# succinctlabs/kzg-rs

Hardware: AMD Instinct MI355X
Metric: blobs/sec verify_blob_kzg_proof_batch (higher is better)
Workload: dtype u32 limbs (255-bit Fr / 381-bit Fp modular integers); 1 GPU; verify_blob_kzg_proof_batch, batches of 1024 synthetic blobs (4096 Fr each), device-resident, known-tau test setup (BASELINE.json configs[1]); one step = one launch group of 256 independent batches = 262144 blobs per GPU; blobs_per_gpu_per_batch=1024, batch=1024, parallelism=shard-by-blob x1, groups_in_flight=4

## Files before the change

### kzg_rs_amd/csrc/capi_verify.hpp

```cpp

static KzgRet launch_evaluate(const KzgSettings* s, const void* d_blobs, const Fr* d_z, Fr* d_y, uint32_t* d_status, size_t T, bool alone = false,
                              bool stamp = false) {
    unsigned long long* const kt = stamp && s->ws.d_ktime ? s->ws.d_ktime + 4 : nullptr;
    if (T > s->eval_scratch_cap) {
        if (s->d_eval_scratch) HIPCHK(hipFree(s->d_eval_scratch));
        s->d_eval_scratch = nullptr;
        s->eval_scratch_cap = 0;
        const size_t cap = T < 1024 ? 1024 : T;
        HIPCHK(hipMalloc(&s->d_eval_scratch, 4 * (size_t)EVAL_SCRATCH_WORDS * cap));
        s->eval_scratch_cap = cap;
    }
    const unsigned per_lane = (unsigned)((T + 63) / 64);
    hipLaunchKernelGGL(k_eval_powers, dim3(per_lane), dim3(64), 0, s->s1, d_z, s->d_eval_scratch, (int)T);
    const unsigned eval_blocks = (unsigned)((T + EVAL_BLOBS_PER_BLOCK - 1) / EVAL_BLOBS_PER_BLOCK);
    static const long pad_opt = ab_int("eval_lds_pad", -1);
    const size_t lds_pad = pad_opt >= 0 ? (size_t)std::min(120L * 1024, pad_opt) : alone ? 0 : 16384;
    size_t spread_lds = eval_blocks <= (unsigned)s->n_cus ? (size_t)EVAL_SPREAD_LDS : lds_pad;
    if (spread_lds && DYN_LDS(k_blob_evaluate_t<true>, spread_lds) != hipSuccess) {
        (void)hipGetLastError();
        spread_lds = 0;
    }
    hipLaunchKernelGGL(k_blob_evaluate_t<true>, dim3(eval_blocks), dim3(64 * EVAL_BLOBS_PER_BLOCK), spread_lds, s->s1,
                       (const uint8_t*)d_blobs, EvalTables{s->d_eval_a, s->d_eval_b, s->d_eval_c}, s->d_eval_scratch, d_status, (int)T, kt);
    hipLaunchKernelGGL(k_eval_finish, dim3(per_lane), dim3(64), 0, s->s1, s->d_eval_scratch, d_y, (int)T);
// ... 127 lines not shown
    MsmDesc d{};
    d.mult = w.d_mult;
    d.pflag = w.d_pflag;
    d.scalars = w.d_scalars;
    d.term_point = w.d_term_point;
    d.term_scalar = w.d_term_scalar;
    d.sorted = w.d_sorted;
    d.window_sums = w.d_window;
    d.nterms[0] = (int)n;
    d.nterms[1] = (int)(2 * n + 1);
    d.max_terms = mt;
    d.stride = 2 * T + 1;
    d.ktime = w.kstamps_valid ? w.d_ktime + 8 : nullptr;
    d.chunks = w.chunks;
    d.chunks_per_block = w.chunks == MSM_CHUNKS ? msm_chunks_per_block(B) : 1;
    static const int msm_flags = ab_flag("msm_xcd", true) ? MSM_FLAG_XCD : 0;
    d.flags = msm_flags;
    const unsigned slots = d.chunks / d.chunks_per_block, W = MSM_WINDOWS / d.chunks;
    unsigned S = 1;
    while (S < MSM_MAX_SLICES && W * slots * 2 * B * S < 768 && n / (2 * S) >= 1024 && 2 * S * B <= 128) S *= 2;
    static const unsigned latency_slices = [] {
        const unsigned v = (unsigned)ab_int("msm_latency_slices", 0);
        return v == 1 || v == 2 || v == 4 || v == 8 ? v : 4u;
    }();
    if (d.chunks != MSM_CHUNKS && S == 1 && n >= 256 && B <= 4) S = latency_slices;
    const size_t lds_cap = msm_lds_sort_capacity<Curve29>();
    auto slice_terms = [&](unsigned S_) { return ((size_t)mt + S_ - 1) / S_ * (size_t)d.chunks_per_block; };
    while (S < MSM_MAX_SLICES && slice_terms(S) > lds_cap && n / (2 * S) >= 1024 && 2 * S * B <= 128) S *= 2;
    const bool lds_sort = slice_terms(S) + 1 <= lds_cap;
    d.slices = (int)S;
    d.window_sums = S > 1 ? w.d_window_sl : w.d_window;
    HIPCHK(hipEventRecord(s->ev[2], s->s1));
    const int nsc = (int)(B * (2 * n + 1));
    hipLaunchKernelGGL(k_glv_split, dim3((unsigned)((nsc + 255) / 256)), dim3(256), 0, s->s1, w.d_scalars, nsc);
    const unsigned gz = (unsigned)(2 * B * S);
    KzgRet rc_save = msm_save_reserve(s, W, slots, gz);
    if (rc_save != KZG_OK) return rc_save;
    if (w.mult_affine) {
        if (lds_sort) msm_window_launch<Curve29Aff, true>(d, W, slots, gz, w.d_msm_save, w.cap_msm_save, s->s1);
        else msm_window_launch<Curve29Aff, false>(d, W, slots, gz, w.d_msm_save, w.cap_msm_save, s->s1);
    } else {
        static const bool tree_quads = ab_flag("msm_tree_quads", true);
        if (tree_quads && d.chunks != MSM_CHUNKS && B <= 4) {
            if (lds_sort) msm_window_launch<Curve29Quads, true>(d, W, slots, gz, w.d_msm_save, w.cap_msm_save, s->s1);
            else msm_window_launch<Curve29Quads, false>(d, W, slots, gz, w.d_msm_save, w.cap_msm_save, s->s1);
        } else if (lds_sort) msm_window_launch<Curve29, true>(d, W, slots, gz, w.d_msm_save, w.cap_msm_save, s->s1);
        else msm_window_launch<Curve29, false>(d, W, slots, gz, w.d_msm_save, w.cap_msm_save, s->s1);
    }
    static const bool sum_quads = ab_flag("msm_sum_quads", true);
    if (sum_quads && W == 1 && slots * S >= 2 && slots * S <= (unsigned)SUMQ_MAX_POINTS && 2 * B < 64) {
        HIPCHK(DYN_LDS(k_msm_sum_quads, SUMQ_LDS_BYTES));
        hipLaunchKernelGGL(k_msm_sum_quads, dim3((unsigned)(2 * B)), dim3(256), SUMQ_LDS_BYTES, s->s1, d.window_sums, w.d_ab, (int)(slots * S));
        HIPCHK(hipGetLastError());
        HIPCHK(hipEventRecord(s->ev[3], s->s1));
        return KZG_OK;
    }
    if (S > 1)
        hipLaunchKernelGGL(k_msm_fold_slices, dim3((unsigned)(2 * B * slots * W)), dim3(64), 0, s->s1, w.d_window_sl, w.d_window, (int)S, (int)W);
    if (2 * B >= 64)
        hipLaunchKernelGGL(k_msm_combine_lanes, dim3((unsigned)((2 * B + 63) / 64)), dim3(64), 0, s->s1, w.d_window, w.d_ab, (int)slots, (int)W, (int)(2 * B));
    else
        hipLaunchKernelGGL(k_msm_combine, dim3((unsigned)(2 * B)), dim3(64), 0, s->s1, w.d_window, w.d_ab, (int)slots, (int)W);
    HIPCHK(hipGetLastError());
    HIPCHK(hipEventRecord(s->ev[3], s->s1));
    return KZG_OK;
}

static KzgRet launch_decode(const KzgSettings* s, const void* d_commitments, const void* d_proofs, size_t T, bool behind_sha = true) {
    Workspace& w = s->ws;
    const int np = (int)(2 * T + 1);
    unsigned blocks = (unsigned)((2 * T + 63) / 64);
    static const bool no_latency_layout = !ab_flag("msm_latency_layout", true);
// ... 1132 lines not shown
```

### kzg_rs_amd/csrc/msm.hpp

```cpp
#pragma once
#include <algorithm>
#include "dyn_lds.hpp"
#include "g1.hpp"
#include "g1_29.hpp"

namespace kzg {

constexpr int MSM_C = 8;
constexpr int MSM_WINDOWS = 32;
constexpr int MSM_BUCKETS = 256;

struct MsmTerm {
    uint32_t point;
};

__global__ __launch_bounds__(256) void k_batch_scalars(const Fr* __restrict__ r_plain, const Fr* __restrict__ zs,
                                                       const Fr* __restrict__ ys, Fr* __restrict__ scalars,
                                                       Fr* __restrict__ partial, int n, unsigned long long offset) {
    __shared__ Fr red[256];
    const int bt = blockIdx.y;
    int i = blockIdx.x * blockDim.x + threadIdx.x;
    zs += (size_t)bt * n;
    ys += (size_t)bt * n;
    Fr* a_out = scalars + (size_t)bt * (2 * n + 1);
    Fr* b_out = a_out + n;
    partial += (size_t)bt * gridDim.x;
    Fr acc = FrF::zero();
    if (i < n) {
        Fr r = FrF::to_mont(r_plain[bt]);
        Fr rp = FrF::one();
        unsigned long long e = offset + (unsigned long long)i;
        for (int b = 63 - __clzll(e | 1ull); b >= 0; b--) {
            rp = FrF::sqr(rp);
            if ((e >> b) & 1) rp = FrF::mul(rp, r);
        }
        a_out[i] = FrF::from_mont(rp);
        b_out[i] = FrF::mul(rp, zs[i]);
        acc = FrF::mul(rp, FrF::to_mont(ys[i]));
    }
    red[threadIdx.x] = acc;
    __syncthreads();
    for (int s = 128; s > 0; s >>= 1) {
        if ((int)threadIdx.x < s) red[threadIdx.x] = FrF::add(red[threadIdx.x], red[threadIdx.x + s]);
        __syncthreads();
    }
    if (threadIdx.x == 0) partial[blockIdx.x] = red[0];
}

__global__ void k_finish_g(const Fr* __restrict__ partial, int nparts, Fr* __restrict__ scalars, int n) {
    if (threadIdx.x) return;
    const int bt = blockIdx.x;
    Fr s = FrF::zero();
    for (int i = 0; i < nparts; i++) s = FrF::add(s, partial[(size_t)bt * nparts + i]);
    scalars[(size_t)bt * (2 * n + 1) + 2 * n] = FrF::from_mont(FrF::neg(s));
}

constexpr int MSM_CHUNKS = 4;
constexpr int MSM_CHUNKS_LATENCY = 32;
constexpr int MSM_ENTRY_CHUNK_SHIFT = 27;
constexpr uint32_t MSM_ENTRY_POINT_MASK = (1u << MSM_ENTRY_CHUNK_SHIFT) - 1;
__device__ __forceinline__ G1Jac g1_neg_phi(const G1Jac& p) {
    G1Jac r;
    r.x = fp_mul(p.x, fp_const(consts::FP_BETA_MONT));
    r.y = fp_neg(p.y);
    r.z = p.z;
    return r;
}
__global__ __launch_bounds__(64, 4) void k_g1_multiples(const G1Aff* __restrict__ points, const uint32_t* __restrict__ pflag,
                                                     G1Jac* __restrict__ mult, int n, int stride, int chunks) {
    int i = blockIdx.x * blockDim.x + threadIdx.x;
    if (i >= n) return;
    const int half = chunks / 2, step = 256 / chunks;
    G1Jac acc = pflag[i] ? g1_identity() : g1_from_affine(points[i]);
    for (int j = 0; j < half; j++) {
        mult[(size_t)j * stride + i] = acc;
        mult[(size_t)(half + j) * stride + i] = g1_neg_phi(acc);
        if (j + 1 < half)
            for (int k = 0; k < step; k++) acc = g1_dbl(acc);
    }
}

__device__ unsigned long long g_decode_dbg[4];

#ifndef KZG_DECODE_OCC
#define KZG_DECODE_OCC 2
#endif
template <int CHUNKS, bool AFF>
__global__ __launch_bounds__(256, KZG_DECODE_OCC) void k_g1_decode_multiples29(const uint8_t* __restrict__ bytes0, const uint8_t* __restrict__ bytes1,
                                                                 int n0, G1Aff* __restrict__ points, uint32_t* __restrict__ pflag,
                                                                 void* __restrict__ mult_, G1Jac29Mem* __restrict__ jtmp, int n, int stride,
                                                                 unsigned long long* __restrict__ ktime = nullptr) {
    static_assert(!AFF || CHUNKS == 4, "the affine layout has one Jacobian multiple per point");
    constexpr int HALF = CHUNKS / 2, STEP = 256 / CHUNKS;
// ... 118 lines not shown
#pragma unroll
    for (int j = 0; j < 4; j++) q[j] = (prod[11 + j] >> 31) | (prod[12 + j] << 1);
    uint32_t ql[8];
#pragma unroll
    for (int j = 0; j < 8; j++) ql[j] = 0;
#pragma unroll
    for (int a = 0; a < 4; a++) {
        uint64_t c = 0;
#pragma unroll
        for (int b = 0; b < 4; b++) {
            uint64_t t = (uint64_t)q[a] * consts::GLV_L[b] + ql[a + b] + c;
            ql[a + b] = (uint32_t)t;
            c = t >> 32;
        }
        ql[a + 4] = (uint32_t)c;
    }
    uint32_t rem[5], borrow = 0;
#pragma unroll
    for (int j = 0; j < 5; j++) rem[j] = subb(k.l[j], ql[j], borrow);
    uint32_t d[5], bo = 0;
#pragma unroll
    for (int j = 0; j < 5; j++) d[j] = subb(rem[j], j < 4 ? consts::GLV_L[j] : 0u, bo);
    const bool ge = bo == 0;
    uint32_t carry = ge ? 1u : 0u;
    Fr out;
#pragma unroll
    for (int j = 0; j < 4; j++) {
        out.l[j] = ge ? d[j] : rem[j];
        out.l[4 + j] = addc(q[j], 0u, carry);
    }
    scalars[i] = out;
}

struct MsmDesc {
    const void* mult;
    const uint32_t* pflag;
    const Fr* scalars;
    const uint32_t* term_point;
    const uint32_t* term_scalar;
    uint32_t* sorted;
    G1Jac* window_sums;
    int nterms[2];
    int max_terms;
    int stride;
    int slices;
    int chunks;
    uint32_t* save;
    int z0;
    int flags;
    unsigned long long* ktime;
    int chunks_per_block;
};

constexpr int MSM_SAVE2_WORDS = 48;
constexpr int MSM_FLAG_ROTATE = 1, MSM_FLAG_XCD = 2, MSM_FLAG_BFIRST = 4;

__device__ __forceinline__ void lds_store_jac(uint32_t* base, int slot, const G1Jac& p) {
    uint32_t* d = base + slot * 36;
#pragma unroll
    for (int i = 0; i < 12; i++) {
        d[i] = p.x.l[i];
        d[12 + i] = p.y.l[i];
        d[24 + i] = p.z.l[i];
    }
}
__device__ __forceinline__ G1Jac lds_load_jac(const uint32_t* base, int slot) {
// ... 264 lines not shown
    if (i == 0) {
        g_decode_dbg[0] = __builtin_amdgcn_s_getreg((31 << 11) | 4);
        g_decode_dbg[1] = __builtin_amdgcn_s_getreg((31 << 11) | 20);
    }
}

__device__ __forceinline__ void lds_store_jac29(uint32_t* base, int slot, const G1Jac29& p) {
    uint32_t* d = base + slot * 42;
#pragma unroll
    for (int i = 0; i < 14; i++) {
        d[i] = p.x.l[i];
        d[14 + i] = p.y.l[i];
        d[28 + i] = p.z.l[i];
    }
}
__device__ __forceinline__ G1Jac29 lds_load_jac29(const uint32_t* base, int slot) {
    const uint32_t* d = base + slot * 42;
    G1Jac29 p;
#pragma unroll
    for (int i = 0; i < 14; i++) {
        p.x.l[i] = d[i];
        p.y.l[i] = d[14 + i];
        p.z.l[i] = d[28 + i];
    }
    return p;
}

struct Curve29 {
    using Pt = G1Jac29;
    using Mem = G1Jac29Mem;
    using Entry = G1Jac29;
    static constexpr int WORDS = 42;
    static constexpr bool QUADS = false;
    using EntryHead = G1AddHead;
    __device__ static __forceinline__ EntryHead entry_head(const Pt& a, const Entry& b) {
        Fp29 Z1Z1, Z2Z2;
        bool p_inf, q_inf;
        g1j29_inf_flags(a, b, Z1Z1, Z2Z2, p_inf, q_inf);
        EntryHead h = g1j29_add_head(a, b, Z1Z1, Z2Z2);
        if (p_inf | q_inf) h.HH = fp29_zero();
        return h;
    }
    __device__ static __forceinline__ bool entry_special(const EntryHead& h) { return g1j29_add_same_x(h); }
    __device__ static __forceinline__ Pt entry_tail(const Pt&, const Entry&, const EntryHead& h) { return g1j29_add_tail(h); }
    __device__ static __forceinline__ Pt from_entry(const Entry& b) { return b; }
    __device__ static __forceinline__ Pt add_entry(const Pt& a, const Entry& b) { return g1j29_add(a, b); }
    __device__ static __forceinline__ Pt identity() { return g1j29_identity(); }
    __device__ static __forceinline__ Pt add(const Pt& a, const Pt& b) { return g1j29_add(a, b); }
    __device__ static __forceinline__ Pt dbl(const Pt& a) { return g1j29_dbl(a); }
    __device__ static __forceinline__ Pt load(const Mem& m) { return g1j29_load(m); }
    __device__ static __forceinline__ void lds_store(uint32_t* b, int s, const Pt& p) { lds_store_jac29(b, s, p); }
    __device__ static __forceinline__ Pt lds_load(const uint32_t* b, int s) { return lds_load_jac29(b, s); }
    __device__ static __forceinline__ G1Jac to_std(const Pt& p) { return g1j29_to_std(p); }
};

struct Curve29Quads : Curve29 {
    static constexpr bool QUADS = true;
};
constexpr size_t MSM_QUADS_LDS_BYTES = 4 * (64 * SUMQ_SCRATCH_WORDS + 32 * Curve29::WORDS + 64 * Curve29::WORDS);
constexpr uint32_t MSM_QUADS_BUCKET_CAP = 3;

struct Curve29Aff : Curve29 {
    using Mem = G1Aff29Mem;
    using Entry = G1Aff29;
    using EntryHead = G1MaddHead;
    __device__ static __forceinline__ EntryHead entry_head(const Pt& a, const Entry& b) { return g1j29_madd_head(a, b); }
    __device__ static __forceinline__ bool entry_special(const EntryHead& h) { return g1j29_madd_special(h); }
    __device__ static __forceinline__ Pt entry_tail(const Pt& a, const Entry&, const EntryHead& h) { return g1j29_madd_tail(a, h); }
    __device__ static __forceinline__ Pt from_entry(const Entry& b) {
        Pt r;
        r.x = b.x;
        r.y = b.y;
        r.z = fp29_const(cp29::FP29_ONE);
        return r;
    }
    __device__ static __forceinline__ Pt add_entry(const Pt& a, const Entry& b) { return g1j29_add_affine(a, b); }
    __device__ static __forceinline__ Entry load(const Mem& m) { return g1a29_load(m); }
};

#ifndef KZG_MSM_OCC
#define KZG_MSM_OCC 3
#endif
template <class CV>
constexpr int msm_lds_sort_capacity() { return MSM_BUCKETS * CV::WORDS; }
template <bool SAFE>
__device__ __forceinline__ G1Jac29 g1j29_add_fast(const G1Jac29& x, const G1Jac29& y, bool& same_x_seen) {
    if constexpr (SAFE) {
        return g1j29_add(x, y);
    } else {
        Fp29 Z1Z1, Z2Z2;
        bool p_inf, q_inf;
        g1j29_inf_flags(x, y, Z1Z1, Z2Z2, p_inf, q_inf);
        if (p_inf | q_inf) return p_inf ? y : x;
        const G1AddHead h = g1j29_add_head(x, y, Z1Z1, Z2Z2);
        same_x_seen |= g1j29_add_same_x(h);
        return g1j29_add_tail(h);
    }
}
template <class CV>
constexpr bool msm_two_pass() { return !CV::QUADS; }
template <class CV, bool LDSSORT = false>
__global__ __launch_bounds__(256, CV::QUADS ? 1 : KZG_MSM_OCC) void k_msm_window(MsmDesc d) {
    using Pt = typename CV::Pt;
    constexpr bool TWOPASS = msm_two_pass<CV>();
    kstamp_in(d.ktime);
    int zz = (int)blockIdx.z + d.z0;
    int w = blockIdx.x;
    if ((d.flags & MSM_FLAG_XCD) && gridDim.x == 8 && gridDim.y == 1 && (gridDim.z & 7) == 0) {
        const unsigned L = blockIdx.x + 8u * blockIdx.z, i = L >> 3;
        w = (int)(i & 7);
        zz = (int)((i >> 3) * 8 + (L & 7)) + d.z0;
    }
    if (d.flags & MSM_FLAG_BFIRST) {
        const int half = (int)(gridDim.z >> 1);
        zz = zz < half ? 2 * zz + 1 : 2 * (zz - half);
    }
    const int S = d.slices, bo = zz / S, slice = zz % S;
    const int o = bo & 1, tid = threadIdx.x;
    const int cpb = d.chunks_per_block, j0 = blockIdx.y * cpb;
    const int W = gridDim.x;
    const int wi = ((bo * gridDim.y + blockIdx.y) * S + slice) * W + w;
    const int t0 = (int)((long long)d.nterms[o] * slice / S), nt = (int)((long long)d.nterms[o] * (slice + 1) / S) - t0;
    const uint32_t* tp = d.term_point + (size_t)bo * d.max_terms + t0;
    const uint32_t* tsc = d.term_scalar + (size_t)bo * d.max_terms + t0;
    __shared__ uint32_t cnt[MSM_BUCKETS], off[MSM_BUCKETS + 1], cur[MSM_BUCKETS];
    __shared__ uint32_t long_buckets[MSM_BUCKETS], n_long;
    extern __shared__ __attribute__((aligned(16))) uint32_t msm_dyn_lds[];
    __shared__ uint32_t pts[TWOPASS ? 1 : MSM_BUCKETS * CV::WORDS];
    uint32_t* const lst = TWOPASS ? msm_dyn_lds : pts;
    uint32_t* const sorted_global = d.sorted + ((size_t)(bo * gridDim.y + blockIdx.y) * W + w) * cpb * d.max_terms + (size_t)cpb * t0;
    cnt[tid] = 0;
    cur[tid] = 0;
    if (tid == 0) n_long = 0;
    __syncthreads();
    const uint8_t* sb = reinterpret_cast<const uint8_t*>(d.scalars);

    for (int c = 0; c < cpb; c++) {
        const int byte = W * (j0 + c) + w;
        for (int t = tid; t < nt; t += 256) {
            uint32_t dig = d.pflag[tp[t]] ? 0u : sb[(size_t)tsc[t] * 32 + byte];
            atomicAdd(&cnt[dig], 1u);
        }
    }
    __syncthreads();
    if (tid == 0) {
        uint32_t s = 0;
        for (int b = 0; b < MSM_BUCKETS; b++) {
            off[b] = s;
            s += cnt[b];
        }
        off[MSM_BUCKETS] = s;
    }
    __syncthreads();
    for (int c = 0; c < cpb; c++) {
        const int byte = W * (j0 + c) + w;
        for (int t = tid; t < nt; t += 256) {
            uint32_t dig = d.pflag[tp[t]] ? 0u : sb[(size_t)tsc[t] * 32 + byte];
            uint32_t pos = atomicAdd(&cur[dig], 1u);
            if constexpr (LDSSORT) lst[off[dig] + pos] = tp[t] | (uint32_t)(j0 + c) << MSM_ENTRY_CHUNK_SHIFT;
            else sorted_global[off[dig] + pos] = tp[t] | (uint32_t)(j0 + c) << MSM_ENTRY_CHUNK_SHIFT;
        }
    }
    __threadfence_block();
    __syncthreads();
    {
        const uint32_t mine = tid ? cnt[tid] : 0u;
        uint32_t rank = 0;
        for (int b = 0; b < MSM_BUCKETS; b++) {
            const uint32_t c = b ? cnt[b] : 0u;
            rank += (c > mine) | ((c == mine) & (b < tid));
        }
        cur[rank] = tid;
    }
    __syncthreads();
    const int rot = (d.flags & MSM_FLAG_ROTATE) ? (int)((blockIdx.x + blockIdx.z) & 3) : 0;
    const int bucket = cur[(tid + 64 * rot) & 255];
    const typename CV::Mem* mult = static_cast<const typename CV::Mem*>(d.mult);
    auto sorted_at = [&](uint32_t k) -> uint32_t {
        if constexpr (LDSSORT) return lst[k];
        else return sorted_global[k];
    };
    auto sorted_put = [&](uint32_t k, uint32_t v) {
        if constexpr (LDSSORT) lst[k] = v;
        else sorted_global[k] = v;
    };
    Pt acc = CV::identity();
    if constexpr (TWOPASS) {
        auto accumulate = [&](uint32_t k, const uint32_t kend) -> Pt {
            Pt a = CV::identity();
            const uint32_t first = k + 1;
            uint32_t wr = k;
            if (k < kend) {
                const uint32_t e = sorted_at(k++);
                a = CV::from_entry(CV::load(mult[(size_t)(e >> MSM_ENTRY_CHUNK_SHIFT) * d.stride + (e & MSM_ENTRY_POINT_MASK)]));
                wr = k;
            }
            for (; k < kend; k++) {
                const uint32_t e = sorted_at(k);
                const typename CV::Entry q = CV::load(mult[(size_t)(e >> MSM_ENTRY_CHUNK_SHIFT) * d.stride + (e & MSM_ENTRY_POINT_MASK)]);
                const typename CV::EntryHead h = CV::entry_head(a, q);
                if (CV::entry_special(h)) sorted_put(wr++, e);
                else a = CV::entry_tail(a, q, h);
            }
            for (uint32_t j = first; j < wr; j++) {
                const uint32_t e = sorted_at(j);
                a = CV::add_entry(a, CV::load(mult[(size_t)(e >> MSM_ENTRY_CHUNK_SHIFT) * d.stride + (e & MSM_ENTRY_POINT_MASK)]));
            }
            return a;
        };
        const size_t slot = ((size_t)(zz - d.z0) * gridDim.y + blockIdx.y) * W + w;
        uint32_t* const out = d.save + slot * MSM_SAVE2_WORDS * 256;
        auto put = [&](int col, const Pt& p) {
            uint4* const o4 = reinterpret_cast<uint4*>(out + (size_t)col * MSM_SAVE2_WORDS);
            const Fp29* const c[3] = {&p.x, &p.y, &p.z};
#pragma unroll
            for (int j = 0; j < 3; j++) {
                o4[4 * j] = make_uint4(c[j]->l[0], c[j]->l[1], c[j]->l[2], c[j]->l[3]);
                o4[4 * j + 1] = make_uint4(c[j]->l[4], c[j]->l[5], c[j]->l[6], c[j]->l[7]);
                o4[4 * j + 2] = make_uint4(c[j]->l[8], c[j]->l[9], c[j]->l[10], c[j]->l[11]);
                o4[4 * j + 3] = make_uint4(c[j]->l[12], c[j]->l[13], 0u, 0u);
            }
        };
        put(bucket, accumulate(bucket > 0 ? off[bucket] : 0u, bucket > 0 ? off[bucket + 1] : 0u));
        kstamp_out(d.ktime);
        return;
    } else {
        uint32_t k = bucket > 0 ? off[bucket] : 0u, w = k;
        const uint32_t kend_all = bucket > 0 ? off[bucket + 1] : 0u;
        const uint32_t kend = (CV::QUADS && kend_all - k > MSM_QUADS_BUCKET_CAP) ? k + MSM_QUADS_BUCKET_CAP : kend_all;
        if (k < kend) {
            const uint32_t e = sorted_at(k++);
            acc = CV::from_entry(CV::load(mult[(size_t)(e >> MSM_ENTRY_CHUNK_SHIFT) * d.stride + (e & MSM_ENTRY_POINT_MASK)]));
            w = k;
        }
        for (; k < kend; k++) {
            const uint32_t e = sorted_at(k);
            const typename CV::Entry q = CV::load(mult[(size_t)(e >> MSM_ENTRY_CHUNK_SHIFT) * d.stride + (e & MSM_ENTRY_POINT_MASK)]);
            const typename CV::EntryHead h = CV::entry_head(acc, q);
            if (CV::entry_special(h)) sorted_put(w++, e);
            else acc = CV::entry_tail(acc, q, h);
        }
        const uint32_t first = bucket > 0 ? off[bucket] + 1 : 0u;
        for (uint32_t j = first; j < w; j++) {
            const uint32_t e = sorted_at(j);
            acc = CV::add_entry(acc, CV::load(mult[(size_t)(e >> MSM_ENTRY_CHUNK_SHIFT) * d.stride + (e & MSM_ENTRY_POINT_MASK)]));
        }
        if constexpr (CV::QUADS) {
            if (kend < kend_all) {
                if constexpr (LDSSORT)
                    for (uint32_t j = kend; j < kend_all; j++) sorted_global[j] = lst[j];
                long_buckets[atomicAdd(&n_long, 1u)] = (uint32_t)bucket;
            }
        }
    }
    if constexpr (LDSSORT) __syncthreads();
    CV::lds_store(pts, bucket, acc);
// ... 96 lines not shown
        __syncthreads();
        if (active) {
            Fp29 Z1Z1, Z2Z2;
            bool p_inf, q_inf;
            g1j29_inf_flags(x, y, Z1Z1, Z2Z2, p_inf, q_inf);
            if (p_inf | q_inf) {
                CV::lds_store(arr, dst, p_inf ? y : x);
            } else {
                const G1AddHead h = g1j29_add_head(x, y, Z1Z1, Z2Z2);
                if (g1j29_add_same_x(h)) CV::lds_store(arr, dst, g1j29_add_same_x_result(h));
                else CV::lds_store(arr, dst, g1j29_add_tail(h));
            }
        }
        __syncthreads();
    }
    if constexpr (CV::QUADS) {
        if (tid < 4) g1j29_add_quad<SumqLayout14>(rc, rc + 16 * CV::WORDS, rc, msm_dyn_lds, tid, tid);
        if (tid < 3) {
            const Fp c = fp29_to_std(SumqLayout14::ld(rc, tid));
            G1Jac& o = d.window_sums[wi];
            *(tid == 0 ? &o.x : tid == 1 ? &o.y : &o.z) = c;
        }
    } else {
        if (tid == 0) {
            Pt r = CV::lds_load(rc, 0);
#pragma unroll 1
            for (int k = 0; k < 4; k++) r = CV::dbl(r);
            d.window_sums[wi] = CV::to_std(CV::add(r, CV::lds_load(rc, 16)));
        }
    }
    kstamp_out(d.ktime);
}

__device__ __forceinline__ G1Jac29 g1j29_shfl(const G1Jac29& p, int src_lane) {
    G1Jac29 r;
#pragma unroll
    for (int i = 0; i < 14; i++) {
        r.x.l[i] = (uint32_t)__shfl((int)p.x.l[i], src_lane, 64);
        r.y.l[i] = (uint32_t)__shfl((int)p.y.l[i], src_lane, 64);
        r.z.l[i] = (uint32_t)__shfl((int)p.z.l[i], src_lane, 64);
    }
    return r;
}
template <bool SAFE>
__global__ __launch_bounds__(256, SAFE ? 1 : 2) void k_msm_reduce(const uint32_t* __restrict__ save, uint32_t* __restrict__ flags,
                                                                    G1Jac* __restrict__ window_sums, int W, int gy, int S, int z0, int nslots) {
    const int tid = threadIdx.x, lane = tid & 63, l = tid & 31;
    int q = (int)blockIdx.x * 8 + (tid >> 5);
    const bool live = q < nslots;
    if (!live) q = nslots - 1;
    if constexpr (SAFE) {
        if (!__any((int)flags[q])) return;
    }
    bool bad = false;
    const bool is_col = l >= 16;
    const int k = l & 15;
    const uint32_t* base = save + (size_t)q * MSM_SAVE2_WORDS * 256;
    G1Jac29 acc = g1j29_identity();
#pragma unroll 1
    for (int t = 0; t < 16; t++) {
        const int b = is_col ? 16 * t + k : 16 * k + t;
        const uint4* const i4 = reinterpret_cast<const uint4*>(base + (size_t)b * MSM_SAVE2_WORDS);
        G1Jac29 pnt;
        Fp29* const c[3] = {&pnt.x, &pnt.y, &pnt.z};
#pragma unroll
        for (int j = 0; j < 3; j++) {
            const uint4 a = i4[4 * j], bb = i4[4 * j + 1], cc = i4[4 * j + 2], dd = i4[4 * j + 3];
            c[j]->l[0] = a.x; c[j]->l[1] = a.y; c[j]->l[2] = a.z; c[j]->l[3] = a.w;
            c[j]->l[4] = bb.x; c[j]->l[5] = bb.y; c[j]->l[6] = bb.z; c[j]->l[7] = bb.w;
            c[j]->l[8] = cc.x; c[j]->l[9] = cc.y; c[j]->l[10] = cc.z; c[j]->l[11] = cc.w;
            c[j]->l[12] = dd.x; c[j]->l[13] = dd.y;
        }
        acc = t == 0 ? pnt : g1j29_add_fast<SAFE>(acc, pnt, bad);
    }
#pragma unroll 1
    for (int s = 1; s < 16; s <<= 1) {
        const G1Jac29 other = g1j29_shfl(acc, (lane + s) & 63);
        if (k + s < 16) acc = g1j29_add_fast<SAFE>(acc, other, bad);
    }
    if (k == 0) acc = g1j29_identity();
#pragma unroll 1
    for (int s = 8; s >= 1; s >>= 1) {
        const G1Jac29 other = g1j29_shfl(acc, (lane + s) & 63);
        if (k < s) acc = g1j29_add_fast<SAFE>(acc, other, bad);
    }
    const G1Jac29 colsum = g1j29_shfl(acc, (lane + 16) & 63);
    if (l == 0) {
#pragma unroll 1
        for (int i = 0; i < 4; i++) acc = g1j29_dbl(acc);
        acc = g1j29_add_fast<SAFE>(acc, colsum, bad);
    }
    const unsigned long long any_bad = __ballot((int)bad);
    const bool win_bad = ((any_bad >> (lane & 32)) & 0xffffffffull) != 0;
    if (l == 0 && live) {
        if constexpr (!SAFE) flags[q] = win_bad ? 1u : 0u;
        if (SAFE ? flags[q] != 0 : !win_bad) {
            const int w = q % W, by = (q / W) % gy, zz = q / (W * gy) + z0;
            const int bo = zz / S, slice = zz % S;
            window_sums[((size_t)(bo * gy + by) * S + slice) * W + w] = g1j29_to_std(acc);
        }
    }
}

template <class CV, bool LDSSORT>
inline void msm_window_launch(MsmDesc d, unsigned gx, unsigned gy, unsigned gz, uint32_t* save, size_t save_bytes, hipStream_t st, bool with_reduce = true) {
    const size_t layer = (size_t)gx * gy * (256 * (msm_two_pass<CV>() ? MSM_SAVE2_WORDS : CV::WORDS) + 1) * 4;
    unsigned per = (unsigned)std::min<size_t>(gz, std::max<size_t>(1, save_bytes / layer));
    d.save = save;
    if (CV::QUADS)
        (void)DYN_LDS((k_msm_window<CV, LDSSORT>), MSM_QUADS_LDS_BYTES);
    if (msm_two_pass<CV>() && per == gz && d.slices == 1 && (gz & 1) == 0 && d.nterms[1] > d.nterms[0]) d.flags |= MSM_FLAG_BFIRST;
    for (unsigned z = 0; z < gz; z += per) {
        d.z0 = (int)z;
        const unsigned nz = std::min(per, gz - z);
        const size_t list_bytes = (msm_two_pass<CV>() && LDSSORT) ? 4 * ((size_t)d.chunks_per_block * ((size_t)(d.max_terms + d.slices - 1) / d.slices + 1) + 4) : 0;
        hipLaunchKernelGGL((k_msm_window<CV, LDSSORT>), dim3(gx, gy, nz), dim3(256), CV::QUADS ? MSM_QUADS_LDS_BYTES : list_bytes, st, d);
        if constexpr (msm_two_pass<CV>()) {
            if (!with_reduce) continue;
            const int nslots = (int)(gx * gy * nz);
            uint32_t* const flags = save + (size_t)per * gx * gy * 256 * MSM_SAVE2_WORDS;
            hipLaunchKernelGGL(k_msm_reduce<false>, dim3((unsigned)((nslots + 7) / 8)), dim3(256), 0, st, (const uint32_t*)save, flags, d.window_sums, (int)gx,
                               (int)gy, d.slices, (int)z, nslots);
            hipLaunchKernelGGL(k_msm_reduce<true>, dim3((unsigned)((nslots + 7) / 8)), dim3(256), 0, st, (const uint32_t*)save, flags, d.window_sums, (int)gx,
                               (int)gy, d.slices, (int)z, nslots);
        }
    }
}
constexpr size_t msm_save_layer_bytes(unsigned gx, unsigned gy, int words) { return (size_t)gx * gy * (256 * words + 1) * 4; }

__global__ __launch_bounds__(64) void k_msm_fold_slices(const G1Jac* __restrict__ sums, G1Jac* __restrict__ out, int slices, int W) {
    const int gw = blockIdx.x, g = gw / W, w = gw % W, tid = threadIdx.x;
    __shared__ uint32_t pts[64 * 36];
    if (tid < slices) lds_store_jac(pts, tid, sums[((size_t)g * slices + tid) * W + w]);
    int width = 1;
    while (width < slices) width <<= 1;
    __syncthreads();
    for (int half = width >> 1; half >= 1; half >>= 1) {
        const bool active = tid < half && tid + half < slices;
        G1Jac x = g1_identity(), y = g1_identity();
        if (active) {
            x = lds_load_jac(pts, tid);
            y = lds_load_jac(pts, tid + half);
        }
        __syncthreads();
        if (active) lds_store_jac(pts, tid, g1_add(x, y));
        __syncthreads();
    }
    if (tid == 0) out[(size_t)g * W + w] = lds_load_jac(pts, 0);
}

__global__ __launch_bounds__(64) void k_msm_combine(const G1Jac* __restrict__ window_sums, G1Jac* __restrict__ out, int nslots, int W) {
    const int o = blockIdx.x, tid = threadIdx.x;
    __shared__ uint32_t pts[32 * 36];
    const int total = nslots * W;
    if (tid < total) lds_store_jac(pts, tid, window_sums[o * total + tid]);
    __syncthreads();
    for (int half = nslots >> 1; half >= 1; half >>= 1) {
// ... 38 lines not shown
    if (tid < 3) {
        const Fp c = fp29_to_std(sumq_load(pts + 16 * tid));
        Fp* dst = tid == 0 ? &out[o].x : tid == 1 ? &out[o].y : &out[o].z;
        *dst = c;
    }
}

__global__ __launch_bounds__(64) void k_msm_combine_quad(const G1Jac* __restrict__ window_sums, G1Jac* __restrict__ out, int W) {
    __shared__ __attribute__((aligned(16))) uint32_t pts[(32 + 1) * 48 + SUMQ_SCRATCH_WORDS];
    const int o = blockIdx.x, tid = threadIdx.x, r = tid & 3;
    uint32_t* const acc = pts + 32 * 48;
    uint32_t* const scr = pts + 33 * 48;
    if (tid < 3 * W) {
        const int w = tid / 3, c = tid % 3;
        const G1Jac& p = window_sums[(size_t)o * W + w];
        sumq_store(pts + w * 48 + 16 * c, fp29_from_std(c == 0 ? p.x : c == 1 ? p.y : p.z));
    }
    __syncthreads();
    if (tid >= 4) return;
    if (r < 3) sumq_store(acc + 16 * r, sumq_load(pts + (W - 1) * 48 + 16 * r));
#pragma unroll 1
    for (int w = W - 2; w >= 0; w--) {
#pragma unroll 1
        for (int k = 0; k < MSM_C; k++) g1j29_dbl_quad<SumqLayout16>(acc, acc, scr, r);
        g1j29_add_quad<SumqLayout16>(acc, pts + w * 48, acc, scr, r, tid);
    }
    if (r < 3) {
        const Fp c = fp29_to_std(sumq_load(acc + 16 * r));
        Fp* dst = r == 0 ? &out[o].x : r == 1 ? &out[o].y : &out[o].z;
        *dst = c;
    }
}

__device__ __forceinline__ G1Jac29 save2_load(const uint32_t* p) {
    const uint4* const i4 = reinterpret_cast<const uint4*>(p);
    G1Jac29 pnt;
    Fp29* const c[3] = {&pnt.x, &pnt.y, &pnt.z};
#pragma unroll
    for (int j = 0; j < 3; j++) {
        const uint4 a = i4[4 * j], bb = i4[4 * j + 1], cc = i4[4 * j + 2], dd = i4[4 * j + 3];
        c[j]->l[0] = a.x; c[j]->l[1] = a.y; c[j]->l[2] = a.z; c[j]->l[3] = a.w;
        c[j]->l[4] = bb.x; c[j]->l[5] = bb.y; c[j]->l[6] = bb.z; c[j]->l[7] = bb.w;
        c[j]->l[8] = cc.x; c[j]->l[9] = cc.y; c[j]->l[10] = cc.z; c[j]->l[11] = cc.w;
        c[j]->l[12] = dd.x; c[j]->l[13] = dd.y;
    }
    return pnt;
}
__device__ __forceinline__ void save2_store(uint32_t* p, const G1Jac29& v) {
    sumq_store(p, v.x);
    sumq_store(p + 16, v.y);
    sumq_store(p + 32, v.z);
}
constexpr int MSM_FOLD_MAX_GROUPS = 128;
template <bool SAFE>
__global__ __launch_bounds__(256) void k_msm_bucket_fold(const uint32_t* __restrict__ save, uint32_t* __restrict__ part, uint32_t* __restrict__ flags, int W,
                                                         int Z, int per, int groups, int gp) {
    const int w = blockIdx.x % W, g = blockIdx.x / W, b = threadIdx.x;
    if constexpr (SAFE) {
        if (!flags[blockIdx.x]) return;
    }
    uint32_t* const dst = part + (((size_t)w * 256 + b) * gp + g) * MSM_SAVE2_WORDS;
    if (g >= groups) {
        save2_store(dst, g1j29_identity());
        return;
    }
    const int z0 = g * per, z1 = min(Z, z0 + per);
    bool bad = false;
    G1Jac29 acc = save2_load(save + (((size_t)z0 * W + w) * 256 + b) * MSM_SAVE2_WORDS);
#pragma unroll 1
    for (int z = z0 + 1; z < z1; z++) acc = g1j29_add_fast<SAFE>(acc, save2_load(save + (((size_t)z * W + w) * 256 + b) * MSM_SAVE2_WORDS), bad);
    save2_store(dst, acc);
    if constexpr (!SAFE) {
        if (__any((int)bad) && (threadIdx.x & 63) == 0) flags[blockIdx.x] = 1u;
    }
}
constexpr size_t msm_bucket_sum_lds_bytes(int gp) { return 4 * ((size_t)gp * SUMQ_POINT_WORDS + 16 * SUMQ_SCRATCH_WORDS); }
__global__ __launch_bounds__(64) void k_msm_bucket_sum_quads(const uint32_t* __restrict__ part, uint32_t* __restrict__ out, int gp) {
    extern __shared__ __attribute__((aligned(16))) uint32_t bsum_lds[];
    uint32_t* const pts = bsum_lds;
    const int tid = threadIdx.x, q = tid >> 2, r = tid & 3;
// ... 122 lines not shown
```

Measured before the change: 4.839 million blobs/s.

## Use signed-digit GLV bucket decomposition for affine MSM windows

Adds a signed-digit GLV split that recodes each 8-bit window into a digit in [-128,128], so only 128 buckets are needed and negative digits are handled by negating the point's y. Each bucket is split across two threads to keep all 256 threads busy, and a matching reduce kernel folds the paired half-bucket sums into window sums. The goal is to halve bucket-reduction work and balance per-bucket load. The cost is an extra field negation per entry, more complex recoding, and a new reduction path that could be wrong on carry edge cases.

```diff
diff --git a/kzg_rs_amd/csrc/capi_verify.hpp b/kzg_rs_amd/csrc/capi_verify.hpp
--- a/kzg_rs_amd/csrc/capi_verify.hpp
+++ b/kzg_rs_amd/csrc/capi_verify.hpp
@@ -183,12 +183,14 @@
     d.window_sums = S > 1 ? w.d_window_sl : w.d_window;
     HIPCHK(hipEventRecord(s->ev[2], s->s1));
     const int nsc = (int)(B * (2 * n + 1));
-    hipLaunchKernelGGL(k_glv_split, dim3((unsigned)((nsc + 255) / 256)), dim3(256), 0, s->s1, w.d_scalars, nsc);
+    const bool signed_digits = w.mult_affine && lds_sort;
+    if (signed_digits) hipLaunchKernelGGL(k_glv_split_signed, dim3((unsigned)((nsc + 255) / 256)), dim3(256), 0, s->s1, w.d_scalars, nsc);
+    else hipLaunchKernelGGL(k_glv_split, dim3((unsigned)((nsc + 255) / 256)), dim3(256), 0, s->s1, w.d_scalars, nsc);
     const unsigned gz = (unsigned)(2 * B * S);
     KzgRet rc_save = msm_save_reserve(s, W, slots, gz);
     if (rc_save != KZG_OK) return rc_save;
     if (w.mult_affine) {
-        if (lds_sort) msm_window_launch<Curve29Aff, true>(d, W, slots, gz, w.d_msm_save, w.cap_msm_save, s->s1);
+        if (signed_digits) msm_window_launch<Curve29AffSigned, true>(d, W, slots, gz, w.d_msm_save, w.cap_msm_save, s->s1);
         else msm_window_launch<Curve29Aff, false>(d, W, slots, gz, w.d_msm_save, w.cap_msm_save, s->s1);
     } else {
         static const bool tree_quads = ab_flag("msm_tree_quads", true);
diff --git a/kzg_rs_amd/csrc/msm.hpp b/kzg_rs_amd/csrc/msm.hpp
--- a/kzg_rs_amd/csrc/msm.hpp
+++ b/kzg_rs_amd/csrc/msm.hpp
@@ -3,6 +3,7 @@
 #include "dyn_lds.hpp"
 #include "g1.hpp"
 #include "g1_29.hpp"
+#include "msm_signed.hpp"
 
 namespace kzg {
 
@@ -59,6 +60,7 @@
 constexpr int MSM_CHUNKS_LATENCY = 32;
 constexpr int MSM_ENTRY_CHUNK_SHIFT = 27;
 constexpr uint32_t MSM_ENTRY_POINT_MASK = (1u << MSM_ENTRY_CHUNK_SHIFT) - 1;
+constexpr uint32_t MSM_ENTRY_NEG = 1u << 31;
 __device__ __forceinline__ G1Jac g1_neg_phi(const G1Jac& p) {
     G1Jac r;
     r.x = fp_mul(p.x, fp_const(consts::FP_BETA_MONT));
@@ -243,6 +245,19 @@
     scalars[i] = out;
 }
 
+__global__ __launch_bounds__(256) void k_glv_split_signed(Fr* __restrict__ scalars, int count) {
+    const int i = blockIdx.x * blockDim.x + threadIdx.x;
+    if (i >= count) return;
+    const Fr k = scalars[i];
+    uint8_t dg[32];
+    glv_split_signed(k.l, dg);
+    Fr out;
+#pragma unroll
+    for (int j = 0; j < 8; j++)
+        out.l[j] = (uint32_t)dg[4 * j] | (uint32_t)dg[4 * j + 1] << 8 | (uint32_t)dg[4 * j + 2] << 16 | (uint32_t)dg[4 * j + 3] << 24;
+    scalars[i] = out;
+}
+
 struct MsmDesc {
     const void* mult;
     const uint32_t* pflag;
@@ -573,6 +588,7 @@
     using Entry = G1Jac29;
     static constexpr int WORDS = 42;
     static constexpr bool QUADS = false;
+    static constexpr bool SIGNED = false;
     using EntryHead = G1AddHead;
     __device__ static __forceinline__ EntryHead entry_head(const Pt& a, const Entry& b) {
         Fp29 Z1Z1, Z2Z2;
@@ -617,6 +633,10 @@
     }
     __device__ static __forceinline__ Pt add_entry(const Pt& a, const Entry& b) { return g1j29_add_affine(a, b); }
     __device__ static __forceinline__ Entry load(const Mem& m) { return g1a29_load(m); }
+};
+
+struct Curve29AffSigned : Curve29Aff {
+    static constexpr bool SIGNED = true;
 };
 
 #ifndef KZG_MSM_OCC
@@ -676,10 +696,18 @@
     __syncthreads();
     const uint8_t* sb = reinterpret_cast<const uint8_t*>(d.scalars);
 
+    auto key_of = [](uint32_t byte) -> uint32_t {
+        if constexpr (CV::SIGNED) return (byte & 0x80u) ? 256u - byte : byte;
+        else return byte;
+    };
+    auto neg_of = [](uint32_t byte) -> uint32_t {
+        if constexpr (CV::SIGNED) return (byte & 0x80u) ? MSM_ENTRY_NEG : 0u;
+        else return 0u;
+    };
     for (int c = 0; c < cpb; c++) {
         const int byte = W * (j0 + c) + w;
         for (int t = tid; t < nt; t += 256) {
-            uint32_t dig = d.pflag[tp[t]] ? 0u : sb[(size_t)tsc[t] * 32 + byte];
+            uint32_t dig = d.pflag[tp[t]] ? 0u : key_of(sb[(size_t)tsc[t] * 32 + byte]);
             atomicAdd(&cnt[dig], 1u);
         }
     }
@@ -696,26 +724,31 @@
     for (int c = 0; c < cpb; c++) {
         const int byte = W * (j0 + c) + w;
         for (int t = tid; t < nt; t += 256) {
-            uint32_t dig = d.pflag[tp[t]] ? 0u : sb[(size_t)tsc[t] * 32 + byte];
+            const uint32_t sbyte = d.pflag[tp[t]] ? 0u : sb[(size_t)tsc[t] * 32 + byte], dig = key_of(sbyte);
             uint32_t pos = atomicAdd(&cur[dig], 1u);
-            if constexpr (LDSSORT) lst[off[dig] + pos] = tp[t] | (uint32_t)(j0 + c) << MSM_ENTRY_CHUNK_SHIFT;
-            else sorted_global[off[dig] + pos] = tp[t] | (uint32_t)(j0 + c) << MSM_ENTRY_CHUNK_SHIFT;
+            const uint32_t e = tp[t] | (uint32_t)(j0 + c) << MSM_ENTRY_CHUNK_SHIFT | neg_of(sbyte);
+            if constexpr (LDSSORT) lst[off[dig] + pos] = e;
+            else sorted_global[off[dig] + pos] = e;
         }
     }
     __threadfence_block();
     __syncthreads();
-    {
-        const uint32_t mine = tid ? cnt[tid] : 0u;
+    constexpr int NB = CV::SIGNED ? MSM_BUCKETS / 2 : MSM_BUCKETS;
+    if (!CV::SIGNED || (tid >= 1 && tid <= NB)) {
+        const uint32_t mine = CV::SIGNED ? cnt[tid] : tid ? cnt[tid] : 0u;
         uint32_t rank = 0;
-        for (int b = 0; b < MSM_BUCKETS; b++) {
-            const uint32_t c = b ? cnt[b] : 0u;
-            rank += (c > mine) | ((c == mine) & (b < tid));
+        for (int b = 0; b < NB; b++) {
+            const int bb = CV::SIGNED ? b + 1 : b;
+            const uint32_t c = bb ? cnt[bb] : 0u;
+            rank += (c > mine) | ((c == mine) & (bb < tid));
         }
         cur[rank] = tid;
     }
     __syncthreads();
     const int rot = (d.flags & MSM_FLAG_ROTATE) ? (int)((blockIdx.x + blockIdx.z) & 3) : 0;
-    const int bucket = cur[(tid + 64 * rot) & 255];
+    const int rslot = (tid + 64 * rot) & 255;
+    const int bucket = CV::SIGNED ? (int)cur[rslot >> 1] : (int)cur[rslot];
+    const int half = CV::SIGNED ? rslot & 1 : 0;
     const typename CV::Mem* mult = static_cast<const typename CV::Mem*>(d.mult);
     auto sorted_at = [&](uint32_t k) -> uint32_t {
         if constexpr (LDSSORT) return lst[k];
@@ -727,25 +760,35 @@
     };
     Pt acc = CV::identity();
     if constexpr (TWOPASS) {
+        auto entry = [&](uint32_t e) -> typename CV::Entry {
+            if constexpr (CV::SIGNED) {
+                const uint32_t u = e & ~MSM_ENTRY_NEG;
+                typename CV::Entry q = CV::load(mult[(size_t)(u >> MSM_ENTRY_CHUNK_SHIFT) * d.stride + (u & MSM_ENTRY_POINT_MASK)]);
+                if (e & MSM_ENTRY_NEG) q.y = fp29_neg<3>(q.y);
+                return q;
+            } else {
+                return CV::load(mult[(size_t)(e >> MSM_ENTRY_CHUNK_SHIFT) * d.stride + (e & MSM_ENTRY_POINT_MASK)]);
+            }
+        };
         auto accumulate = [&](uint32_t k, const uint32_t kend) -> Pt {
             Pt a = CV::identity();
             const uint32_t first = k + 1;
             uint32_t wr = k;
             if (k < kend) {
                 const uint32_t e = sorted_at(k++);
-                a = CV::from_entry(CV::load(mult[(size_t)(e >> MSM_ENTRY_CHUNK_SHIFT) * d.stride + (e & MSM_ENTRY_POINT_MASK)]));
+                a = CV::from_entry(entry(e));
                 wr = k;
             }
             for (; k < kend; k++) {
                 const uint32_t e = sorted_at(k);
-                const typename CV::Entry q = CV::load(mult[(size_t)(e >> MSM_ENTRY_CHUNK_SHIFT) * d.stride + (e & MSM_ENTRY_POINT_MASK)]);
+                const typename CV::Entry q = entry(e);
                 const typename CV::EntryHead h = CV::entry_head(a, q);
                 if (CV::entry_special(h)) sorted_put(wr++, e);
                 else a = CV::entry_tail(a, q, h);
             }
             for (uint32_t j = first; j < wr; j++) {
                 const uint32_t e = sorted_at(j);
-                a = CV::add_entry(a, CV::load(mult[(size_t)(e >> MSM_ENTRY_CHUNK_SHIFT) * d.stride + (e & MSM_ENTRY_POINT_MASK)]));
+                a = CV::add_entry(a, entry(e));
             }
             return a;
         };
@@ -762,7 +805,12 @@
                 o4[4 * j + 3] = make_uint4(c[j]->l[12], c[j]->l[13], 0u, 0u);
             }
         };
-        put(bucket, accumulate(bucket > 0 ? off[bucket] : 0u, bucket > 0 ? off[bucket + 1] : 0u));
+        if constexpr (CV::SIGNED) {
+            const uint32_t lo = off[bucket], hi = off[bucket + 1], mid = lo + (hi - lo + 1) / 2;
+            put(2 * (bucket - 1) + half, accumulate(half ? mid : lo, half ? hi : mid));
+        } else {
+            put(bucket, accumulate(bucket > 0 ? off[bucket] : 0u, bucket > 0 ? off[bucket + 1] : 0u));
+        }
         kstamp_out(d.ktime);
         return;
     } else {
@@ -925,6 +973,20 @@
     kstamp_out(d.ktime);
 }
 
+__device__ __forceinline__ G1Jac29 save2_load(const uint32_t* p) {
+    const uint4* const i4 = reinterpret_cast<const uint4*>(p);
+    G1Jac29 pnt;
+    Fp29* const c[3] = {&pnt.x, &pnt.y, &pnt.z};
+#pragma unroll
+    for (int j = 0; j < 3; j++) {
+        const uint4 a = i4[4 * j], bb = i4[4 * j + 1], cc = i4[4 * j + 2], dd = i4[4 * j + 3];
+        c[j]->l[0] = a.x; c[j]->l[1] = a.y; c[j]->l[2] = a.z; c[j]->l[3] = a.w;
+        c[j]->l[4] = bb.x; c[j]->l[5] = bb.y; c[j]->l[6] = bb.z; c[j]->l[7] = bb.w;
+        c[j]->l[8] = cc.x; c[j]->l[9] = cc.y; c[j]->l[10] = cc.z; c[j]->l[11] = cc.w;
+        c[j]->l[12] = dd.x; c[j]->l[13] = dd.y;
+    }
+    return pnt;
+}
 __device__ __forceinline__ G1Jac29 g1j29_shfl(const G1Jac29& p, int src_lane) {
     G1Jac29 r;
 #pragma unroll
@@ -991,6 +1053,50 @@
             const int w = q % W, by = (q / W) % gy, zz = q / (W * gy) + z0;
             const int bo = zz / S, slice = zz % S;
             window_sums[((size_t)(bo * gy + by) * S + slice) * W + w] = g1j29_to_std(acc);
+        }
+    }
+}
+
+template <bool SAFE>
+__global__ __launch_bounds__(256, SAFE ? 1 : 2) void k_msm_reduce_signed(const uint32_t* __restrict__ save, uint32_t* __restrict__ flags,
+                                                                           G1Jac* __restrict__ window_sums, int W, int gy, int S, int z0, int nslots) {
+    const int tid = threadIdx.x, lane = tid & 63, k = tid & 15;
+    int q = (int)blockIdx.x * 16 + (tid >> 4);
+    const bool live = q < nslots;
+    if (!live) q = nslots - 1;
+    if constexpr (SAFE) {
+        if (!__any((int)flags[q])) return;
+    }
+    bool bad = false;
+    const uint32_t* const base = save + ((size_t)q * 256 + (size_t)16 * k) * MSM_SAVE2_WORDS;
+    G1Jac29 run = g1j29_identity(), wsum = g1j29_identity();
+#pragma unroll 1
+    for (int t = 15; t >= 0; t--) {
+        const G1Jac29 pnt = save2_load(base + (size_t)t * MSM_SAVE2_WORDS);
+        run = t == 15 ? pnt : g1j29_add_fast<SAFE>(run, pnt, bad);
+        if ((t & 1) == 0) wsum = t == 14 ? run : g1j29_add_fast<SAFE>(wsum, run, bad);
+    }
+#pragma unroll 1
+    for (int s = 1; s < 16; s <<= 1) {
+        const G1Jac29 other = g1j29_shfl(run, (lane + s) & 63);
+        if (k + s < 16) run = g1j29_add_fast<SAFE>(run, other, bad);
+    }
+#pragma unroll 1
+    for (int i = 0; i < 3; i++) run = g1j29_dbl(run);
+    if (k > 0) wsum = g1j29_add_fast<SAFE>(wsum, run, bad);
+#pragma unroll 1
+    for (int s = 8; s >= 1; s >>= 1) {
+        const G1Jac29 other = g1j29_shfl(wsum, (lane + s) & 63);
+        if (k < s) wsum = g1j29_add_fast<SAFE>(wsum, other, bad);
+    }
+    const unsigned long long any_bad = __ballot((int)bad);
+    const bool win_bad = ((any_bad >> (lane & 48)) & 0xffffull) != 0;
+    if (k == 0 && live) {
+        if constexpr (!SAFE) flags[q] = win_bad ? 1u : 0u;
+        if (SAFE ? flags[q] != 0 : !win_bad) {
+            const int w = q % W, by = (q / W) % gy, zz = q / (W * gy) + z0;
+            const int bo = zz / S, slice = zz % S;
+            window_sums[((size_t)(bo * gy + by) * S + slice) * W + w] = g1j29_to_std(wsum);
         }
     }
 }
@@ -1012,10 +1118,17 @@
             if (!with_reduce) continue;
             const int nslots = (int)(gx * gy * nz);
             uint32_t* const flags = save + (size_t)per * gx * gy * 256 * MSM_SAVE2_WORDS;
-            hipLaunchKernelGGL(k_msm_reduce<false>, dim3((unsigned)((nslots + 7) / 8)), dim3(256), 0, st, (const uint32_t*)save, flags, d.window_sums, (int)gx,
-                               (int)gy, d.slices, (int)z, nslots);
-            hipLaunchKernelGGL(k_msm_reduce<true>, dim3((unsigned)((nslots + 7) / 8)), dim3(256), 0, st, (const uint32_t*)save, flags, d.window_sums, (int)gx,
-                               (int)gy, d.slices, (int)z, nslots);
+            if constexpr (CV::SIGNED) {
+                hipLaunchKernelGGL(k_msm_reduce_signed<false>, dim3((unsigned)((nslots + 15) / 16)), dim3(256), 0, st, (const uint32_t*)save, flags, d.window_sums,
+                                   (int)gx, (int)gy, d.slices, (int)z, nslots);
+                hipLaunchKernelGGL(k_msm_reduce_signed<true>, dim3((unsigned)((nslots + 15) / 16)), dim3(256), 0, st, (const uint32_t*)save, flags, d.window_sums,
+                                   (int)gx, (int)gy, d.slices, (int)z, nslots);
+            } else {
+                hipLaunchKernelGGL(k_msm_reduce<false>, dim3((unsigned)((nslots + 7) / 8)), dim3(256), 0, st, (const uint32_t*)save, flags, d.window_sums,
+                                   (int)gx, (int)gy, d.slices, (int)z, nslots);
+                hipLaunchKernelGGL(k_msm_reduce<true>, dim3((unsigned)((nslots + 7) / 8)), dim3(256), 0, st, (const uint32_t*)save, flags, d.window_sums,
+                                   (int)gx, (int)gy, d.slices, (int)z, nslots);
+            }
         }
     }
 }
@@ -1120,20 +1233,6 @@
     }
 }
 
-__device__ __forceinline__ G1Jac29 save2_load(const uint32_t* p) {
-    const uint4* const i4 = reinterpret_cast<const uint4*>(p);
-    G1Jac29 pnt;
-    Fp29* const c[3] = {&pnt.x, &pnt.y, &pnt.z};
-#pragma unroll
-    for (int j = 0; j < 3; j++) {
-        const uint4 a = i4[4 * j], bb = i4[4 * j + 1], cc = i4[4 * j + 2], dd = i4[4 * j + 3];
-        c[j]->l[0] = a.x; c[j]->l[1] = a.y; c[j]->l[2] = a.z; c[j]->l[3] = a.w;
-        c[j]->l[4] = bb.x; c[j]->l[5] = bb.y; c[j]->l[6] = bb.z; c[j]->l[7] = bb.w;
-        c[j]->l[8] = cc.x; c[j]->l[9] = cc.y; c[j]->l[10] = cc.z; c[j]->l[11] = cc.w;
-        c[j]->l[12] = dd.x; c[j]->l[13] = dd.y;
-    }
-    return pnt;
-}
 __device__ __forceinline__ void save2_store(uint32_t* p, const G1Jac29& v) {
     sumq_store(p, v.x);
     sumq_store(p + 16, v.y);
diff --git a/kzg_rs_amd/csrc/msm_signed.hpp b/kzg_rs_amd/csrc/msm_signed.hpp
--- /dev/null
+++ b/kzg_rs_amd/csrc/msm_signed.hpp
@@ -0,0 +1,111 @@
+#pragma once
+#include <stdint.h>
+
+#if defined(__HIPCC__)
+#define MSMS_FN __host__ __device__ __forceinline__
+#else
+#define MSMS_FN inline
+#endif
+
+namespace kzg {
+namespace cglv {
+#define KZG_CONST static constexpr
+#include "constants.inc"
+#undef KZG_CONST
+}
+
+template <int N>
+MSMS_FN void msms_sub(uint32_t* r, const uint32_t* a, const uint32_t* b) {
+    uint64_t br = 0;
+#pragma unroll
+    for (int i = 0; i < N; i++) {
+        const uint64_t t = (uint64_t)a[i] - b[i] - br;
+        r[i] = (uint32_t)t;
+        br = (t >> 63) & 1;
+    }
+}
+template <int N>
+MSMS_FN void msms_add_small(uint32_t* r, int32_t c) {
+    uint64_t t = (uint64_t)r[0] + (uint32_t)c;
+    r[0] = (uint32_t)t;
+    const uint32_t ext = c < 0 ? 0xffffffffu : 0u;
+#pragma unroll
+    for (int i = 1; i < N; i++) {
+        t = (t >> 32) + r[i] + ext;
+        r[i] = (uint32_t)t;
+    }
+}
+template <int N>
+MSMS_FN bool msms_gt(const uint32_t* a, const uint32_t* b) {
+    uint64_t br = 0;
+#pragma unroll
+    for (int i = 0; i < N; i++) br = (((uint64_t)b[i] - a[i] - br) >> 63) & 1;
+    return br != 0;
+}
+
+MSMS_FN void glv_split_signed(const uint32_t* k, uint8_t* digits) {
+    uint32_t prod[16];
+#pragma unroll
+    for (int j = 0; j < 16; j++) prod[j] = 0;
+#pragma unroll
+    for (int a = 0; a < 8; a++) {
+        uint64_t c = 0;
+#pragma unroll
+        for (int b = 0; b < 8; b++) {
+            const uint64_t t = (uint64_t)k[a] * cglv::GLV_M[b] + prod[a + b] + c;
+            prod[a + b] = (uint32_t)t;
+            c = t >> 32;
+        }
+        prod[a + 8] = (uint32_t)c;
+    }
+    uint32_t k2[5], ql[5], k1[5], Lw[5], h[5];
+#pragma unroll
+    for (int j = 0; j < 4; j++) k2[j] = (prod[11 + j] >> 31) | (prod[12 + j] << 1);
+    k2[4] = 0;
+#pragma unroll
+    for (int j = 0; j < 5; j++) ql[j] = 0;
+#pragma unroll
+    for (int a = 0; a < 4; a++) {
+        uint64_t c = 0;
+#pragma unroll
+        for (int b = 0; b < 4; b++) {
+            if (a + b >= 5) continue;
+            const uint64_t t = (uint64_t)k2[a] * cglv::GLV_L[b] + ql[a + b] + c;
+            ql[a + b] = (uint32_t)t;
+            c = t >> 32;
+        }
+        if (a + 4 < 5) ql[a + 4] = (uint32_t)c;
+    }
+    msms_sub<5>(k1, k, ql);
+#pragma unroll
+    for (int j = 0; j < 4; j++) Lw[j] = cglv::GLV_L[j];
+    Lw[4] = 0;
+    if (!msms_gt<5>(Lw, k1)) {
+        msms_sub<5>(k1, k1, Lw);
+        msms_add_small<5>(k2, 1);
+    }
+#pragma unroll
+    for (int j = 0; j < 5; j++) h[j] = (Lw[j] >> 1) | (j < 4 ? Lw[j + 1] << 31 : 0u);
+    if (msms_gt<5>(k1, h)) {
+        msms_sub<5>(k1, k1, Lw);
+        msms_add_small<5>(k2, 1);
+    }
+    if (msms_gt<5>(k2, h)) {
+        msms_sub<5>(k2, k2, Lw);
+        msms_add_small<5>(k2, 1);
+        msms_add_small<5>(k1, -1);
+    }
+#pragma unroll
+    for (int half = 0; half < 2; half++) {
+        const uint32_t* v = half ? k2 : k1;
+        uint32_t c = 0;
+#pragma unroll
+        for (int j = 0; j < 16; j++) {
+            const uint32_t b = ((v[j >> 2] >> (8 * (j & 3))) & 0xffu) + c;
+            c = b >= 128u ? 1u : 0u;
+            digits[16 * half + j] = (uint8_t)b;
+        }
+    }
+}
+
+}
```

Result: faster. 4.887 million blobs/s, median of 6 (+1.0%).
